# nmtrmail/Graphite

Hardware: AMD Instinct MI355X
Metric: simulated mem accesses/sec (node) at 1024 tiles, 1/2/4/8 GPU; bit-exact stats (higher is better)
Workload: dtype u64; 1 GPU; configs[3]: 1024 tiles (32x32 mesh) x 256 accesses per tile of the hotspot trace (20% to 256 lines shared by all tiles, WRITE p=1/3, ~2-cycle gaps), pr_l1_pr_l2_dram_directory_msi + full-map directory + DRAM history-tree queue + emesh_hop_by_hop (history-tree router contention), quantum 1000 ns, 8 logical shards (2-D blocks) over 1 GPU(s); tiles=1024, accesses_per_tile=256, hot_lines=256, mode=coherent, network=hop_by_hop

## Files before the change

graphite_amd/csrc/gg_coh_dev.h:

```cpp
#pragma once
#include "gg_dev.h"

#include <algorithm>
#include <type_traits>
#include <cmath>
#include <cstring>
#include <cstdlib>
#include <vector>

#ifndef GG_COH_DIAG
#define GG_COH_DIAG 0
#endif
#define DG(x) (GG_COH_DIAG ? (x) : nullptr)

namespace ggc {
using namespace gg;

enum { M_EX_REQ = GG_MSG_EX_REQ, M_SH_REQ = GG_MSG_SH_REQ, M_INV_REQ = GG_MSG_INV_REQ,
       M_FLUSH_REQ = GG_MSG_FLUSH_REQ, M_WB_REQ = GG_MSG_WB_REQ, M_EX_REP = GG_MSG_EX_REP,
       M_SH_REP = GG_MSG_SH_REP, M_INV_REP = GG_MSG_INV_REP, M_FLUSH_REP = GG_MSG_FLUSH_REP,
       M_WB_REP = GG_MSG_WB_REP, M_NULLIFY_REQ = GG_MSG_NULLIFY_REQ };
enum { DS_UNCACHED = 0, DS_SHARED = 1, DS_MODIFIED = 2, DS_OWNED = 3  };
enum { ST_I = 0, ST_S = 1, ST_M = 2, ST_O = 3  };
enum { M_UPGRADE_REP = GG_MSG_UPGRADE_REP, M_IFC_REQ = GG_MSG_INV_FLUSH_COMBINED_REQ };
enum { M_DRAM_FETCH_REQ = GG_MSG_DRAM_FETCH_REQ, M_DRAM_STORE_REQ = GG_MSG_DRAM_STORE_REQ,
       M_DRAM_FETCH_REP = GG_MSG_DRAM_FETCH_REP,
       M_DOWNGRADE_REQ = GG_MSG_DOWNGRADE_REQ, M_SH_REP_EX = GG_MSG_SH_REP_EX,
       M_DOWNGRADE_REP = GG_MSG_DOWNGRADE_REP };
constexpr uint32_t ST_E = ST_O;
enum { P_SELF = 0, P_LEFT, P_RIGHT, P_DOWN, P_UP, P_INJ };
#define INV_ADDR (~0ull)
#define NO_ENT (-0x7fffffff)

__device__ __forceinline__ bool to_directory(uint32_t t)
{
  return t == M_EX_REQ || t == M_SH_REQ || t == M_INV_REP || t == M_FLUSH_REP || t == M_WB_REP;
}
__device__ __forceinline__ bool has_data(uint32_t t)
{
  return t == M_EX_REP || t == M_SH_REP || t == M_FLUSH_REP || t == M_WB_REP ||
         t == M_DRAM_STORE_REQ || t == M_DRAM_FETCH_REP ||
         t == M_SH_REP_EX;
}
__device__ __forceinline__ uint32_t len_class(uint32_t t) { return has_data(t) ? 1u : t == M_IFC_REQ ? 2u : 0u; }

struct DEnt { uint64_t addr; int32_t owner; uint16_t dstate; uint16_t nsh; };
struct HMsg { uint64_t addr, arrival_ps; uint32_t type, src, requester, single_rx; };
struct TileSt { uint64_t rec, rec_end, clk, pend_start, out_addr, out_time; uint32_t blocked, seq, nrep, nrq; };
static_assert(sizeof(TileSt) == 64, "one 64-B line per tile");
struct CReq { uint64_t addr, time; uint32_t type, requester; };
struct CReqX { uint64_t arrival, start; uint32_t ds0, upg; int32_t sharer; uint32_t pad; };
constexpr uint32_t kCdl = 64;
constexpr uint64_t kRng0 = ((uint64_t)(uint32_t)GG_MOSI_RNG_SEED << 16) | 0x330Eu;
#define GG_LDS __attribute__((address_space(3)))
#define GG_GLB __attribute__((address_space(1)))
#if defined(__HIP_DEVICE_COMPILE__)
#define GG_DP __attribute__((address_space(1)))
#else
#define GG_DP
#endif
template <class D, class Q> inline void cs_set(D& dst, Q src) { dst = (D)src; }
struct Seg { uint32_t line, lo, hi, pad; };
enum { QS_Q = 0, QS_START, QS_DONE, QS_ARRIVED, QS_ACTIVE, QS_BLOCKED, QS_MIN_NEXT, QS_COUNT, QS_QPS,
       QS_BWAIT, QS_BMAX, QS_REL, QS_STOP, QS_N };
constexpr uint64_t kQsPaused = 4;
constexpr uint32_t kBarWait = 2;
__device__ __forceinline__ uint64_t rec_gap(uint32_t meta)
{
  return meta == GG_META_BARRIER ? 0ull : (uint64_t)((meta & 0x7FFFFFFFu) >> 1);
}

constexpr uint32_t kInLds = 512;
constexpr uint32_t kRqLds = 512;
constexpr uint32_t kChunks = 128;
constexpr uint32_t kChunk = 16;
constexpr uint32_t kQMax = 128;
constexpr uint32_t kNetCtr = 7;
constexpr size_t kWalkLdsMax = 160 * 1024;
constexpr uint32_t kWalkPkBytes = 5 * 8 + 7 * 4;

struct CP {
  uint32_t T, K, L;
  uint32_t s1, a1, s2, a2, log_line, pol1, pol2;
  uint32_t E, dassoc, log_dsets, log_slices, W, R, QC, IC;
  uint32_t bits_req, bits_data, bits_ifc, max_list, analytical, dram_qm, dram_qtype, dram_qaux;
  uint32_t net, nsx, nsy, mw, mh, qimg;
  uint32_t msg_cap, seg_cap, walk_pk;
  uint32_t seg_xcd;
  uint32_t cache_lds_off, cache_lds_bytes;
  uint32_t touch_each;
  uint32_t walk_wide;
  uint32_t no_hit_runs;
  uint32_t mt1, mt2, mt_log;
  uint32_t fast;
  uint32_t mosi;
  uint32_t shl2;
  uint32_t mesi;
  uint64_t lat_l1d, lat_l1t, lat_l2d, lat_l2t, lat_dir, gap_ps, dram_proc, dram_cost;
  NocParams np;
};

__device__ __forceinline__ uint32_t class_bits(const CP& P, uint32_t c) { return c == 1 ? P.bits_data : c == 2 ? P.bits_ifc : P.bits_req; }
__device__ __forceinline__ uint32_t msg_bits(const CP& P, uint32_t t) { return class_bits(P, len_class(t)); }

struct CS {
  GG_DP uint64_t* l1_tag; GG_DP uint8_t* l1_meta; GG_DP uint8_t* l1_rr;
  GG_DP uint64_t* l2_tag; GG_DP uint8_t* l2_meta; GG_DP uint8_t* l2_rr;
  GG_DP uint64_t* cc;
  GG_DP uint64_t* mtab;
  GG_DP unsigned long long* mtc;
  GG_DP uint64_t* st;
  GG_DP TileSt* ts;
  GG_DP DEnt* dir; GG_DP uint64_t* dsh;
  GG_DP DEnt* rep; GG_DP uint64_t* rsh;
  GG_DP CReq* rq;
  GG_DP CReqX* rqx;
  GG_DP uint64_t* drng; GG_DP uint64_t* rrng;
  GG_DP uint64_t* cdl; GG_DP uint32_t* ncdl;
  GG_DP uint64_t* ps;
  GG_DP HQueue* dq; GG_DP HNode* dnd;
  GG_DP const uint32_t* gtile; GG_DP const int32_t* ltile; GG_DP const uint32_t* shard;
  GG_DP const uint4* tinfo;
  GG_DP const uint64_t* addr; GG_DP const uint32_t* meta; GG_DP uint64_t* out;
  GG_DP gg_cmsg* pool0; GG_DP gg_cmsg* pool1; GG_DP uint32_t* npool;
  GG_DP uint32_t* inb0; GG_DP uint32_t* inb1;
  GG_DP uint32_t* arv0; GG_DP uint32_t* arv1;
  GG_DP uint32_t* cnt4;
  GG_DP uint64_t* xl; GG_DP uint32_t* nxl; GG_DP uint64_t* yl; GG_DP uint32_t* nyl;
  GG_DP const Seg* segx; GG_DP const Seg* segy;
  GG_DP const uint32_t* tseg;
  GG_DP gg_cmsg* bnd; GG_DP uint32_t* bnd_cnt;
// ... 2963 lines not shown
    r[20] = _hd; r[21] = _hl; r[22] = _hn;
    for (int i = 0; i < 9; ++i) r[23 + i] = T.tra[i];
  }
  if (T.rec >= T.rec_end) return kNsFin;
  if (T.blocked) return kNsBlk;
  return T.clk + rec_gap(S.meta[T.rec]) * P.gap_ps;
}


__device__ __forceinline__ void diag_off(CS& S)
{
  if (!GG_COH_DIAG) { S.prof = nullptr; S.trs = nullptr; S.trw = nullptr; S.tre = nullptr; }
}

#ifndef GG_KWARM
#define GG_KWARM 1
#endif
template <class A, class B>
__device__ __forceinline__ void kwarm(const A* __restrict__ a, const B* __restrict__ b)
{
  if (!GG_KWARM) return;
  const uint32_t* wa = reinterpret_cast<const uint32_t*>(a);
  const uint32_t* wb = reinterpret_cast<const uint32_t*>(b);
  constexpr uint32_t kA = (uint32_t)((sizeof(A) + 63) / 64), kB = (uint32_t)((sizeof(B) + 63) / 64);
  uint32_t x[kA + kB];
#pragma unroll
  for (uint32_t i = 0; i < kA; ++i) x[i] = wa[16 * i];
#pragma unroll
  for (uint32_t i = 0; i < kB; ++i) x[kA + i] = wb[16 * i];
  uint32_t acc = 0;
#pragma unroll
  for (uint32_t i = 0; i < kA + kB; ++i) acc ^= x[i];
  asm volatile("; kwarm %0" ::"s"(acc));
}

__device__ __forceinline__ void kt_begin(const CS& S)
{
  if (S.kt && threadIdx.x == 0)
    S.kt[(size_t)S.kt_slot * S.kt_stride + 2 * blockIdx.x] = __builtin_amdgcn_s_memrealtime();
}
__device__ __forceinline__ void kt_end(const CS& S)
{
  if (!S.kt) return;
  __syncthreads();
  if (threadIdx.x == 0) S.kt[(size_t)S.kt_slot * S.kt_stride + 2 * blockIdx.x + 1] = __builtin_amdgcn_s_memrealtime();
}


constexpr uint32_t kWalkSync = 512;
constexpr uint32_t kMaxWalkWaves = 16;
#ifndef GG_WALK_SLEEP
#define GG_WALK_SLEEP 1
#endif

__device__ __forceinline__ uint64_t wave_min64(uint64_t v)
{
#pragma unroll
  for (int o = 32; o > 0; o >>= 1) { const uint64_t u = (uint64_t)__shfl_xor((long long)v, o); v = u < v ? u : v; }
  return v;
}
__device__ __forceinline__ uint64_t lds_load_rlx(const uint64_t* p)
{
  return __hip_atomic_load(p, __ATOMIC_RELAXED, __HIP_MEMORY_SCOPE_WORKGROUP);
}
__device__ __forceinline__ void lds_store_rlx(uint64_t* p, uint64_t v)
{
  __hip_atomic_store(p, v, __ATOMIC_RELAXED, __HIP_MEMORY_SCOPE_WORKGROUP);
}

__device__ __forceinline__ uint64_t pipe_word(uint64_t t, uint32_t pos, uint32_t status)
{
  return (t << 12) | ((uint64_t)pos << 2) | status;
}
__device__ __forceinline__ uint32_t pipe_pos(uint64_t w) { return (uint32_t)(w >> 2) & 0x3FFu; }

struct WalkLds {
  uint64_t *Pt, *Ph, *Pk, *Pz;
  uint32_t *Pi, *Pp, *Pd, *Pf, *Pr;
  uint64_t *Qt; uint32_t *Qr, *Qs;
};

template <class Q>
__device__ __forceinline__ uint64_t serve_packet(const CP& P, const CS& S, const WalkLds& W, Q&& request, uint32_t i,
                                                 uint32_t nx, const Seg& sd, uint64_t zps, uint64_t& cf)
{
  const uint64_t t = W.Pt[i];
  const uint32_t f = W.Pf[i], nf = f & 0xFFFFFFu, d = W.Pd[i];
  const uint64_t qd = request(t, nf);
  cf += nf;
  uint32_t status = 0;
  if (nx < sd.lo || nx > sd.hi) status = 2;
  else if (nx == d) status = 1;
  W.Pt[i] = t + zps + lat_to_ps(qd, P.np.f);
  W.Pz[i] += zps;
  W.Pf[i] = nf | (status << 24);
  return qd;
}

__host__ __device__ inline bool walk_regq(const CP& P)
{
  return P.np.qm && P.np.qtype == GG_QM_HISTORY_TREE && P.np.max_size <= kQMax;
}

template <bool PIPE, bool RQ>
__device__ __forceinline__ void walk_body(const CP& P, const CS& S, uint32_t L, int stage, uint32_t blk, uint32_t qend = 0)
{
  uint32_t sg = blk;
  if (P.seg_xcd) {
    const uint32_t ns = P.seg_xcd, b = blk;
    sg = 2 * ((b % ns) + ns * (b / (2 * ns))) + ((b / ns) & 1u);
  }
  const uint32_t tid = threadIdx.x, nthr = blockDim.x, ln = tid & 63;
  const uint32_t wv = (uint32_t)__builtin_amdgcn_readfirstlane((int)(tid >> 6));
  uint32_t* cntp = (stage == 0 ? S.nxl : S.nyl) + sg;
  const uint64_t* list = (stage == 0 ? S.xl : S.yl) + (size_t)sg * P.seg_cap;
  const uint32_t live = S.live[L & 3];
  const uint32_t n0 = *cntp;
  const Seg sd = (stage == 0 ? S.segx : S.segy)[sg >> 1];
  const uint64_t lw = tid < P.seg_cap ? list[tid] : 0ull;
  uint32_t sent = 1;
  uint64_t qe_q = 0, qe_Q = 0;
  if (qend) {
    const uint32_t r0 = S.ring[0], r1 = S.ring[1], r2 = S.ring[2], r3 = S.ring[3], i0 = S.imp[0], i1 = S.imp[1];
    qe_q = S.qs[QS_Q]; qe_Q = S.qs[QS_COUNT];
    const uint32_t k = live - 1, km = k & 3;
    sent = (km == 0 ? r0 : km == 1 ? r1 : km == 2 ? r2 : r3) + (k == 0 ? ((qe_Q & 1) ? i1 : i0) : 0u);
  }
  if (!live) return;
  if (sent == 0) { quantum_end_walk(P, S, L, qe_q, qe_Q, blk, qend); return; }
  const uint32_t p = (live - 1) & 1u;
  PROF_T0();
  if (n0 == 0) return;
  const uint32_t n = min(n0, P.seg_cap);
  const uint32_t dir = sg & 1u;
  const int port = stage == 0 ? (dir ? P_RIGHT : P_LEFT) : (dir ? P_UP : P_DOWN);
  auto tile_at = [&](uint32_t pos) -> uint32_t { return stage == 0 ? sd.line * P.mw + pos : pos * P.mw + sd.line; };
  auto pos_of = [&](uint32_t tile) -> uint32_t { return stage == 0 ? tile % P.mw : tile / P.mw; };
  gg_cmsg* cur = pool(S, p);
  extern __shared__ __attribute__((aligned(16))) uint8_t smem[];
  const uint32_t npos = sd.hi - sd.lo + 1;
  const bool qm = RQ || P.np.qm != 0;
  constexpr bool regq = RQ;
  const bool sweep = !PIPE || n > 128 || P.walk_wide;
  const bool direct = PIPE && regq && !sweep;
  RegQueue rq;
  RegQueue::Raw rqr;
  const bool rq_direct = direct && wv < npos;
  const uint64_t rq_qi = rq_direct ? (uint64_t)tile_at(dir ? sd.lo + wv : sd.hi - wv) * 6 + port : 0ull;
  uint8_t* qimg = smem;
  uint64_t* lc = reinterpret_cast<uint64_t*>(smem + (size_t)npos * P.qimg);
  uint32_t* rlohi = reinterpret_cast<uint32_t*>(lc + (size_t)npos * kNetCtr);
  uint8_t* pk = reinterpret_cast<uint8_t*>(rlohi) + kWalkSync;
  if (n > P.walk_pk) { if (tid == 0) { atomicOr(S.err, GG_DERR_CAP); *cntp = 0; } return; }
  WalkLds W;
  W.Pt = reinterpret_cast<uint64_t*>(pk);
  W.Ph = W.Pt + P.walk_pk; W.Pk = W.Ph + P.walk_pk; W.Pz = W.Pk + P.walk_pk;
  W.Pi = reinterpret_cast<uint32_t*>(W.Pz + P.walk_pk);
  W.Pp = W.Pi + P.walk_pk; W.Pd = W.Pp + P.walk_pk; W.Pf = W.Pd + P.walk_pk;
  W.Pr = W.Pf + P.walk_pk;
  W.Qt = reinterpret_cast<uint64_t*>(W.Pr + P.walk_pk);
  W.Qr = reinterpret_cast<uint32_t*>(W.Qt + P.walk_pk); W.Qs = W.Qr + P.walk_pk;
  uint32_t pdst = 0, pf = 0;
  bool pheld = false;
  uint64_t haddr = 0;
  uint32_t hreq = 0, htype = 0, hlink = 0, hsrx = 0;
  const bool has_p = tid < n;
  const uint32_t orec = has_p ? (uint32_t)lw : 0u;
  pdst = has_p ? (uint32_t)(lw >> 32) : 0u;
  const gg_cmsg& om = cur[orec];
  const uint64_t ot = om.arrival_ps, os = om.send_ps, oz = om.zero_load_ps;
  const uint32_t osrc = om.src, oseq = om.seq, ohop = om.hop, otype = om.type;
  haddr = om.addr; hreq = om.requester; hlink = om.link; hsrx = om.single_rx;
  {
    const uint32_t z = pos_of(pdst);
    pheld = has_p && (z < sd.lo || z > sd.hi);
    const uint32_t hx = tile_at(z);
    pf = hx == pdst ? (uint32_t)S.ltile[pdst] : S.tseg[(size_t)hx * 2 + 1];
  }
  if (rq_direct) rqr = RegQueue::issue(S.nq + rq_qi, S.nnd + rq_qi * P.np.max_size, P.np.max_size, ln);
  if (tid < n) {
    const uint32_t i = tid;
    htype = otype;
    W.Pt[i] = ot; W.Ph[i] = os; W.Pk[i] = ((uint64_t)osrc << 32) | oseq; W.Pz[i] = oz;
    W.Pi[i] = orec; W.Pp[i] = pos_of(ohop); W.Pd[i] = pos_of(pdst);
    if (ot >> 51) atomicOr(S.err, GG_DERR_CAP);
    W.Pf[i] = (uint32_t)nflits(P.np, msg_bits(P, otype));
  }
// ... 59 lines not shown
    uint8_t* im = qimg + (size_t)(pos - sd.lo) * P.qimg;
    tr = HTree{reinterpret_cast<HQueue*>(im), reinterpret_cast<HNode*>(im + sizeof(HQueue)), 1, P.np.analytical != 0};
    if (regq) rq.load(tr.q, tr.nd, 1, P.np.analytical != 0, ln);
  };
  auto add_ctr = [&](uint32_t pos, uint64_t cq, uint64_t m, uint64_t cf) {
    uint64_t* l = lc + (size_t)(pos - sd.lo) * kNetCtr;
    l[0] += qm ? cq : 0; l[1] += qm ? m : 0; l[2] += cf; l[3] += m; l[4] += cf; l[5] += cf;
  };
  if (sweep && wv == 0) {
    uint64_t* K = W.Qt; uint32_t* B = W.Qr; uint32_t* O = W.Qs;
    for (uint32_t s_ = 0; lo <= hi && s_ <= hi - lo; ++s_) {
      const uint32_t pos = dir ? lo + s_ : hi - s_;
      uint32_t m = 0;
      for (uint32_t b0 = 0; b0 < n; b0 += 64) {
        const uint32_t i = b0 + ln;
        const bool at = i < n && W.Pp[i] == pos && (W.Pf[i] >> 24) == 0;
        const uint64_t bm = __ballot(at);
        if (at) {
          const uint32_t k = m + (uint32_t)__builtin_popcountll(bm & ((1ull << ln) - 1));
          B[k] = i; K[k] = (W.Pt[i] << 12) | W.Pr[i];
        }
        m += (uint32_t)__builtin_popcountll(bm);
      }
      if (m == 0) continue;
      wave_sync();
      for (uint32_t k = ln; k < m; k += 64) {
        const uint64_t kk = K[k];
        uint32_t r = 0;
        for (uint32_t j = 0; j < m; ++j) r += K[j] < kk;
        O[r] = B[k];
      }
      wave_sync();
      RegQueue rq; HTree tr;
      port_queue(pos, rq, tr);
      auto request = [&](uint64_t t, uint32_t nf) -> uint64_t {
        if (!qm) return 0;
        const uint64_t tc = time_to_cycles(t, P.np.f);
        return regq ? rq.request<false>(tc, nf, S.err) : (wave_q ? tr.delay_w(tc, nf, S.err, ln) : tr.delay(tc, nf, S.err));
      };
      const uint32_t nx = dir ? pos + 1 : pos - 1;
      uint64_t cq = 0, cf = 0;
      for (uint32_t k = 0; k < m; ++k) {
        const uint32_t i = O[k];
        cq += serve_packet(P, S, W, request, i, nx, sd, zps, cf);
        if (ln == 0) W.Pp[i] = nx;
        wave_sync();
      }
      nev += m;
      if (regq) rq.store(tr.q, tr.nd);
      if (ln == 0) add_ctr(pos, cq, m, cf);
      wave_sync();
    }
  } else if (!sweep && wv < npos) {
    const uint32_t pos = dir ? sd.lo + wv : sd.hi - wv;
    const uint32_t nx = dir ? pos + 1 : pos - 1;
    constexpr uint64_t kInf = ~0ull;
    const bool visited = lo <= hi && pos >= lo && pos <= hi;
    HTree tr;
    if (visited && !direct) port_queue(pos, rq, tr);
    const uint32_t status_nx = (nx < sd.lo || nx > sd.hi) ? 2u : 0u;
    const uint64_t zk = zps << 12;
    uint64_t cq = 0, cf = 0, m = 0;
    uint32_t spin = 0, polls = 0;
    const bool tev = DG(S.tre) && L >= kTrEv0 && L < kTrEv0 + S.tre_n;
    unsigned long long* tre = tev ? DG(S.tre) + (((size_t)(L - kTrEv0) * 2 + stage) * S.tr_wb + blk) * (kTrEvMax * 4 + 4) : nullptr;
    auto crosses = [&](uint32_t i) {
      if (i >= n) return false;
      const uint32_t a = W.Pp[i], z = W.Pd[i];
      return dir ? (a <= pos && pos < z) : (a >= pos && pos > z);
    };
    bool c0 = visited && crosses(ln), c1 = visited && crosses(ln + 64);
    const uint32_t r0 = c0 ? W.Pr[ln] : 0u, r1 = c1 ? W.Pr[ln + 64] : 0u;
    const uint32_t fd0 = c0 ? (W.Pf[ln] & 0xFFFFFFu) | (W.Pd[ln] << 24) : 0u;
    const uint32_t fd1 = c1 ? (W.Pf[ln + 64] & 0xFFFFFFu) | (W.Pd[ln + 64] << 24) : 0u;
    uint32_t go = visited ? 1u : 0u;
    uint64_t l0 = kInf, l1 = kInf;
    bool waiting = false;
    while (__builtin_amdgcn_readfirstlane((int)go)) {
      const uint64_t w0 = c0 ? lds_load_rlx(&W.Qt[ln]) : kInf;
      const uint64_t w1 = c1 ? lds_load_rlx(&W.Qt[ln + 64]) : kInf;
      if (waiting && !__ballot(w0 != l0 || w1 != l1)) {
        if (++spin > (1u << 22)) { if (ln == 0) atomicOr(S.err, GG_DERR_STATE); go = 0; continue; }
        __builtin_amdgcn_s_sleep(GG_WALK_SLEEP);
        continue;
      }
      waiting = false;
      l0 = w0; l1 = w1;
      uint64_t mk = kInf, bk = kInf;
      uint32_t mi = 0, mfd = 0;
      if (c0) {
        const uint32_t pp = pipe_pos(w0);
        const uint64_t k = (w0 & ~0xFFFull) | r0;
        if (pp == pos) { mk = k; mi = ln; mfd = fd0; }
        else bk = k + (uint64_t)(dir ? pos - pp : pp - pos) * zk;
      }
      if (c1) {
        const uint32_t pp = pipe_pos(w1);
        const uint64_t k = (w1 & ~0xFFFull) | r1;
        if (pp == pos) {
          if (k < mk) { mk = k; mi = ln + 64; mfd = fd1; }
        } else {
          const uint64_t b = k + (uint64_t)(dir ? pos - pp : pp - pos) * zk;
          bk = b < bk ? b : bk;
        }
      }
      uint64_t wk = kInf;
      uint32_t wl = 0;
      for (uint64_t bm = __ballot(mk != kInf); bm; bm &= bm - 1) {
        const uint32_t l = (uint32_t)__builtin_ctzll(bm);
        const uint64_t k = rl64(mk, l);
        if (k < wk) { wk = k; wl = l; }
      }
      const uint64_t below = __ballot(bk < wk);
      if (wk == kInf && !below) { go = 0; continue; }
      if (below) {
        if (++spin > (1u << 22)) { if (ln == 0) atomicOr(S.err, GG_DERR_STATE); go = 0; continue; }
        ++polls;
        waiting = true;
        __builtin_amdgcn_s_sleep(GG_WALK_SLEEP);
        continue;
      }
      const uint64_t T = wk >> 12;
      const uint64_t ev0 = tev ? __builtin_amdgcn_s_memtime() : 0;
      const uint32_t i = (uint32_t)__builtin_amdgcn_readlane((int)mi, (int)wl);
      const uint32_t fd = (uint32_t)__builtin_amdgcn_readlane((int)mfd, (int)wl);
      const uint32_t nf = fd & 0xFFFFFFu;
      const uint32_t status = status_nx ? status_nx : (nx == (fd >> 24) ? 1u : 0u);
      uint64_t evp = 0;
      auto pub = [&](uint64_t qd) {
        if (tev) evp = __builtin_amdgcn_s_memtime();
        if (ln == 0) lds_store_rlx(&W.Qt[i], pipe_word(T + zps + lat_to_ps(qd, P.np.f), nx, status));
      };
      uint64_t qd = 0;
      if (!qm) pub(0ull);
      else {
        const uint64_t tc = rfl64(time_to_cycles(T, P.np.f));
        if (regq) qd = rq.request_pub(tc, nf, pub);
        else { qd = wave_q ? tr.delay_w(tc, nf, S.err, ln) : tr.delay(tc, nf, S.err); pub(qd); }
      }
      const uint64_t ev1 = tev ? __builtin_amdgcn_s_memtime() : 0;
      cq += qd; cf += nf; ++m;
      if (ln == (i & 63)) { if (i < 64) c0 = false; else c1 = false; }
      if (tev && ln == 0) {
        const uint32_t k = atomicAdd(reinterpret_cast<unsigned int*>(&rlohi[2]), 1u);
        if (k < kTrEvMax) {
          unsigned long long* e = tre + 4 + 4 * k;
          e[0] = ev0; e[1] = evp; e[2] = ev1;
          e[3] = (unsigned long long)i | ((unsigned long long)pos << 16) | ((unsigned long long)wv << 24) |
                 ((unsigned long long)polls << 32);
        }
      }
      wave_sync();
    }
    if (regq && visited && direct && m) {
      const uint64_t qi = (uint64_t)tile_at(pos) * 6 + port;
      rq.errp = S.err; rq.store(S.nq + qi, S.nnd + qi * P.np.max_size);
    } else if (regq && visited && !direct) {
      rq.errp = S.err; rq.store(tr.q, tr.nd);
    }
    if (ln == 0 && visited) add_ctr(pos, cq, m, cf);
    nev = (uint32_t)m;
  }
  if (tid < n) {
    const uint32_t hx = tile_at(pos_of(pdst));
    pself = !pheld && hx == pdst;
    if (pheld) jres = atomicAdd(S.bnd_cnt, 1u);
    else if (pself) jres = atomicAdd(narv_at(S, p ^ 1u, pf), 1u);
    else { s2res = pf * 2 + (pdst / P.mw > hx / P.mw ? 1u : 0u); jres = atomicAdd(&S.nyl[s2res], 1u); }
  }
  __syncthreads();
  PROF_AT(_w2);
  uint32_t nb = 0;
  for (uint32_t i = tid; i < n; i += nthr) {
    const uint32_t r = W.Pi[i];
    uint32_t stt = W.Pf[i] >> 24, p1 = W.Pp[i];
    uint64_t ta = W.Pt[i], z = W.Pz[i];
    gg_cmsg* m = cur + r;
    if (!sweep) {
      const uint64_t w = W.Qt[i];
      const uint32_t p0 = p1;
      ta = w >> 12; p1 = pipe_pos(w); stt = (uint32_t)w & 3u;
      z += (uint64_t)(dir ? p1 - p0 : p0 - p1) * zps;
    }
    const uint32_t h = tile_at(p1);
    m->arrival_ps = ta; m->zero_load_ps = z; m->hop = h;
    const bool own = i == tid;
    if (stt == 2) {
      if (own && !pheld) { atomicOr(S.err, GG_DERR_STATE); continue; }
      const uint32_t j = own ? jres : atomicAdd(S.bnd_cnt, 1u);
      if (j >= P.msg_cap) { atomicOr(S.err, GG_DERR_CAP); continue; }
      gg_cmsg g;
      if (own) {
        const uint64_t kk = W.Pk[i];
        g.addr = haddr; g.send_ps = W.Ph[i]; g.src = (uint32_t)(kk >> 32); g.dst = pdst; g.requester = hreq;
        g.seq = (uint32_t)kk; g.type = htype; g.link = hlink; g.single_rx = hsrx;
      } else {
        g = *m;
      }
      g.arrival_ps = ta; g.zero_load_ps = z; g.hop = h;
      S.bnd[j] = g;
      ++nb;
      continue;
    }
    const uint32_t dst = own ? pdst : m->dst;
    if (own && (pheld || pself != (h == dst))) { atomicOr(S.err, GG_DERR_STATE); continue; }
// ... 198 lines not shown
```

graphite_amd/csrc/gg_coherent.hip:

```cpp
#include "gg_coh_many.h"
#include "gg_stats.h"
#include "gg_snapshot.h"

#include <algorithm>
#include <cmath>
#include <cstring>
#include <vector>

namespace ggc {

__global__ void k_c_import(CP P, CS S, const gg_cmsg* in, uint32_t n)
{
  const uint32_t i = blockIdx.x * blockDim.x + threadIdx.x;
  if (i >= n) return;
  import_one(P, S, in[i], &S.imp[0]);
}

__global__ void k_has_barrier(const uint32_t* meta, uint64_t n, uint32_t* flag)
{
  for (uint64_t i = (uint64_t)blockIdx.x * blockDim.x + threadIdx.x; i < n; i += (uint64_t)gridDim.x * blockDim.x)
    if (meta[i] == GG_META_BARRIER) { *flag = 1; return; }
}

__global__ void k_c_status(CP P, CS S, uint64_t* out )
// ... 936 lines not shown
    GG_HIP(hipGetLastError());
    uint64_t done = 0;
    uint32_t err = 0;
    GG_HIP(hipMemcpyAsync(&done, C->S.qs + QS_DONE, sizeof(done), hipMemcpyDeviceToHost, s));
    GG_HIP(hipMemcpyAsync(&err, ctx->err_dev, sizeof(err), hipMemcpyDeviceToHost, s));
    GG_HIP(hipStreamSynchronize(s));
    timed_harvest(C);
    if (err) break;
    if (done) break;
    if (batch < 256) batch *= 2;
  }
  gg_timer_end(ctx, "coherent_run", s);
  GG_HIP(hipStreamSynchronize(s));
  if (C->S.trs && getenv("GG_COH_TRACE_OUT")) {
    const std::string pre = getenv("GG_COH_TRACE_OUT");
    const size_t ns = (size_t)C->S.tr_n * P.L * kTrStep, nw = (size_t)C->S.tr_n * 2 * C->S.tr_wb * 8;
    std::vector<unsigned long long> h(std::max(ns, nw));
    for (int k = 0; k < 2; ++k) {
      const size_t cnt = k ? nw : ns;
      GG_HIP(hipMemcpy(h.data(), k ? C->S.trw : C->S.trs, 8 * cnt, hipMemcpyDeviceToHost));
      if (FILE* f = fopen((pre + (k ? ".walk" : ".step")).c_str(), "wb")) { fwrite(h.data(), 8, cnt, f); fclose(f); }
    }
    if (C->S.tre) {
      const size_t ne = (size_t)C->S.tre_n * 2 * C->S.tr_wb * (kTrEvMax * 4 + 4);
      std::vector<unsigned long long> he(ne);
      GG_HIP(hipMemcpy(he.data(), C->S.tre, 8 * ne, hipMemcpyDeviceToHost));
      if (FILE* f = fopen((pre + ".ev").c_str(), "wb")) { fwrite(he.data(), 8, ne, f); fclose(f); }
    }
    if (FILE* f = fopen((pre + ".meta").c_str(), "w")) {
      fprintf(f, "{\"launches\": %u, \"tiles\": %u, \"walk_blocks\": %u, \"nsx\": %u, \"nsy\": %u, \"wtx\": %u, \"wty\": %u, "
              "\"ev_first\": %u, \"ev_launches\": %u, \"ev_max\": %u}\n",
              C->S.tr_n, P.L, C->S.tr_wb, P.nsx, P.nsy, C->wtx, C->wty, kTrEv0, C->S.tre_n, kTrEvMax);
      fclose(f);
    }
  }
  if (C->S.prof) {
    std::vector<unsigned long long> h(1024 + 8 * 65536);
    GG_HIP(hipMemcpy(h.data(), C->S.prof, sizeof(unsigned long long) * h.size(), hipMemcpyDeviceToHost));
    unsigned long long crit = 0, wx = 0, wy = 0;
    for (int i = 0; i < 65536; ++i) { crit += h[1024 + i]; wx += h[1024 + 65536 + 2 * i]; wy += h[1024 + 65536 + 2 * i + 1]; }
    fprintf(stderr, "[gg_coh] step cycles over tiles: self %llu inbox+handlers %llu (order %llu) trace %llu publish %llu "
            "writeback %llu | slowest tile per launch %llu\n"
            "[gg_coh] walkers: %llu launches, staging %llu events %llu loop %llu handoff %llu, max events X %llu Y %llu | "
            "slowest walker per launch X %llu Y %llu | sweep: batch %llu queue load %llu requests %llu store %llu (s_memtime cycles); requests fast %llu M/G/1 %llu search %llu\n",
            h[0], h[1], h[9], h[2], h[3], h[4], crit, h[22], h[16], h[19], h[17], h[18], h[24], h[25], wx, wy, h[26], h[27], h[28], h[29], h[30], h[31], h[32]);
    {
      unsigned long long mt = 0, mx = 0, my = 0;
      for (int i = 0; i < 65536; ++i) { mt += h[1024 + 3 * 65536 + i]; mx += h[1024 + 4 * 65536 + 2 * i]; my += h[1024 + 4 * 65536 + 2 * i + 1]; }
      fprintf(stderr, "[gg_coh] tiles with SELF arrivals: %llu; cycles prologue %llu, narv %llu, gather %llu, order %llu, queue load %llu, "
              "requests + store %llu | tiles without: %llu, prologue %llu\n", h[96], h[90], h[91], h[92], h[93], h[94], h[95], h[98], h[97]);
      fprintf(stderr, "[gg_coh] per-launch max requests summed: tile (self+sent) %llu walker X %llu Y %llu\n", mt, mx, my);
      fprintf(stderr, "[gg_coh] walkers: most packets in one run X %llu Y %llu; pipelined runs past 64 packets (a lane's second "
              "candidate; past 128 wave 0 sweeps) %llu\n", h[46], h[47], h[48]);
      unsigned long long sn = 0, sa = 0, ss = 0, c1 = 0, c2 = 0, c3 = 0, ct = 0, nl = 0;
      for (int i = 0; i < 16384; ++i) {
        const unsigned long long* b = &h[1024 + 6 * 65536 + 4 * i];
        if (!b[0]) continue;
        ++nl; ct += b[0] >> 24;
        sn += (b[0] >> 16) & 255; sa += (b[0] >> 8) & 255; ss += b[0] & 255;
        c1 += (b[1] & 0xFFFFFF) << 8; c2 += (b[2] & 0xFFFFFF) << 8; c3 += (b[3] & 0xFFFFFF) << 8;
      }
      fprintf(stderr, "[gg_coh] slowest tile per launch (%llu launches, last 16384 indices): cycles %llu; inbox msgs %llu, SELF arrivals %llu, "
              "sent %llu; cycles self-phase %llu inbox+handlers %llu trace %llu\n", nl, ct, sn, sa, ss, c1, c2, c3);
      const char* kn[3] = {"SELF", "injection", "walker"};
      for (int k = 0; k < 3; ++k)
        fprintf(stderr, "[gg_coh] %s batches, requests by size 1|2-3|4-7|8-15|16-31|32-63|64+: %llu %llu %llu %llu %llu %llu %llu; tail requests %llu\n",
                kn[k], h[50 + 8 * k], h[51 + 8 * k], h[52 + 8 * k], h[53 + 8 * k], h[54 + 8 * k], h[55 + 8 * k], h[56 + 8 * k], h[80 + k]);
    }
    fprintf(stderr, "[gg_coh] trace: hit runs %llu cycles for %llu records (%llu calls, look-up part %llu; %llu row updates: "
            "loop %llu stores %llu); other accesses %llu cycles for %llu\n",
            h[33], h[34], h[38], h[37] - h[39], h[42], h[40] - h[37] + 0, h[41] - h[40], h[35], h[36]);
  }
  if (gg_status e = coh_check(ctx)) return e;
  uint64_t done = 0;
  GG_HIP(hipMemcpy(&done, C->S.qs + QS_DONE, sizeof(done), hipMemcpyDeviceToHost));
  *done_out = done;
  if (done == 2) return gg_fail(GG_ERR_STATE, "coherent run deadlocked: tiles blocked with no message in flight");
  return GG_OK;
}

static gg_status coh_owns_all(const gg_ctx* ctx, gg_status code, const char* what)
{
  const gg_config& c = ctx->cfg;
  const uint32_t K = c.num_shards ? c.num_shards : 1;
  if (c.shard_begin != 0 || (c.shard_end != 0 && c.shard_end != K))
    return gg_fail(code, "%s needs a context that owns every shard", what);
  return GG_OK;
}

gg_status gg_coherent_run(gg_ctx* ctx, const gg_trace* tr, uint64_t* access_out_dev, void* stream)
{
  GG_NOT_ATAC(ctx, "gg_coherent_run");
  if (!ctx) return gg_fail(GG_ERR_INVALID, "NULL argument");
  if (gg_status st = coh_owns_all(ctx, GG_ERR_INVALID, "gg_coherent_run")) return st;
  if (gg_status st = gg_coherent_begin(ctx, tr, access_out_dev, stream)) return st;
  uint64_t done = 0;
  return coh_drive(ctx, true, &done);
}

gg_status gg_coherent_advance(gg_ctx* ctx, uint64_t stop_quantum, uint64_t* next_quantum, int* done)
{
  GG_NOT_ATAC(ctx, "gg_coherent_advance");
  if (!ctx || !next_quantum || !done) return gg_fail(GG_ERR_INVALID, "NULL argument");
  if (gg_status st = coh_owns_all(ctx, GG_ERR_UNSUPPORTED, "gg_coherent_advance")) return st;
  gg_coh_state* C = ctx->coh;
  if (!C || !C->begun) return gg_fail(GG_ERR_INVALID, "gg_coherent_begin or gg_coherent_restore first");
// ... 605 lines not shown
```

graphite_amd/csrc/gg_dev.h:

```cpp
#pragma once
#include "gg_internal.h"

namespace gg {

struct HNode { uint64_t first, second; };
struct HQueue {
  uint32_t size; uint32_t max_size; uint32_t type, aux;
  uint64_t sig_sq, sig, n, newest;
  uint64_t analytical;
  uint64_t util, last_req, total_req;
  uint32_t front, back;
  double mean;
  uint64_t qtime;
  uint32_t head, pad;
};
static_assert(sizeof(HQueue) % 16 == 0 && sizeof(HNode) == 16, "16-byte queue images");

__host__ __device__ inline uint32_t hq_aux(uint32_t type, uint32_t basic_moving_avg, uint32_t list_no_interleaving)
{
  return type == GG_QM_BASIC ? basic_moving_avg : list_no_interleaving;
}
__host__ __device__ inline uint32_t hq_window(uint32_t aux) { return (aux & 0xFFFFu) ? (aux & 0xFFFFu) : 64u; }

inline gg_status gg_check_queue_model(uint32_t type, uint32_t aux, uint32_t max_size)
// ... 499 lines not shown
      } else {
        qd = la - t;
        if (lb - (la + p) >= min_proc) set(i1, la + p, lb);
        else --sz;
      }
    } else if (analytical && A(0) > t + p) {
      ++anl; ++n_anl;
      qd = mg1_queue_delay(nreq, newest, sig_sq, sig);
    } else {
      ++n_gen;
      const uint64_t tp = t + p;
      const uint64_t v0 = low_lanes(sz), v1 = sz > 64 ? low_lanes(sz - 64) : 0ull;
      const uint64_t le0 = cmp64<kCmpULE>(a0, t) & v0, le1 = cmp64<kCmpULE>(a1, t) & v1;
      const uint64_t f0 = le0 & cmp64<kCmpUGE>(b0, tp), f1 = le1 & cmp64<kCmpUGE>(b1, tp);
      const uint64_t l0 = ~le0 & v0 & cmp64<kCmpUGE>(b0 - a0, p), l1 = ~le1 & v1 & cmp64<kCmpUGE>(b1 - a1, p);
      const bool fit = (f0 | f1) != 0;
      const uint64_t m0 = fit ? f0 : l0, m1 = fit ? f1 : l1;
      const int i = m0 ? (int)__builtin_ctzll(m0) : (m1 ? 64 + (int)__builtin_ctzll(m1) : -1);
      if (i < 0) {
        errs |= GG_DERR_STATE;
      } else {
        const uint32_t ui = (uint32_t)i;
        const uint64_t a = A(ui), b = B(ui);
        if (t >= a) {
          if (t - a >= min_proc) {
            if (b - (t + p) >= min_proc) { shift_up(ui + 1); set(ui + 1, t + p, b); ++sz; }
            set(ui, a, t);
          } else if (b - (t + p) >= min_proc) {
            set(ui, t + p, b);
          } else {
            shift_down(ui); --sz;
          }
        } else {
          qd = a - t;
          if (b - (a + p) >= min_proc) set(ui, a + p, b);
          else { shift_down(ui); --sz; }
        }
      }
    }
    sig_sq += p * p;
    sig += p;
    if (sig_sq >= kMg1Exact || p >= (1ull << 26)) errs |= GG_DERR_RANGE;
    ++nreq;
    const uint64_t x = t + qd + p;
    newest = x > newest ? x : newest;
    util += p;
    last_req = x > last_req ? x : last_req;
    ++total_req;
    return qd;
  }
  __device__ __forceinline__ uint64_t rd64(uint64_t v) const { return rfl64(v); }
  __device__ __forceinline__ uint64_t A1(uint32_t i) const { return i < 64 ? rl64(a0, i) : rl64(a1, i - 64); }
  __device__ __forceinline__ uint64_t B1(uint32_t i) const { return i < 64 ? rl64(b0, i) : rl64(b1, i - 64); }
  template <class Pub>
  __device__ __forceinline__ uint64_t request_pub(uint64_t t, uint64_t p, Pub&& pub)
  {
    if (sz >= cap) { shift_down(0); --sz; }
    uint64_t qd = 0;
    const uint64_t tp = t + p;
    const uint64_t v0 = low_lanes(sz), v1 = sz > 64 ? low_lanes(sz - 64) : 0ull;
    const uint64_t le0 = cmp64<kCmpULE>(a0, t) & v0, le1 = cmp64<kCmpULE>(a1, t) & v1;
    const uint64_t f0 = le0 & cmp64<kCmpUGE>(b0, tp), f1 = le1 & cmp64<kCmpUGE>(b1, tp);
    if (f0 | f1) {
      pub(0ull);
      ++n_gen;
      const uint32_t ui = f0 ? (uint32_t)__builtin_ctzll(f0) : 64u + (uint32_t)__builtin_ctzll(f1);
      const uint64_t a = A1(ui), b = B1(ui);
      if (t - a >= min_proc) {
        if (b - tp >= min_proc) { shift_up(ui + 1); set(ui + 1, tp, b); ++sz; }
        set(ui, a, t);
      } else if (b - tp >= min_proc) {
        set(ui, tp, b);
      } else {
        shift_down(ui); --sz;
      }
    } else if (analytical && (cmp64<kCmpUGT>(a0, tp) & 1ull)) {
      qd = mg1_queue_delay(nreq, newest, sig_sq, sig);
      pub(qd);
      ++anl; ++n_anl;
    } else {
      ++n_gen;
      const uint64_t m0 = ~le0 & v0 & cmp64<kCmpUGE>(b0 - a0, p);
      const uint64_t m1 = ~le1 & v1 & cmp64<kCmpUGE>(b1 - a1, p);
      if ((m0 | m1) == 0) {
        pub(0ull);
        errs |= GG_DERR_STATE;
      } else {
        const uint32_t ui = m0 ? (uint32_t)__builtin_ctzll(m0) : 64u + (uint32_t)__builtin_ctzll(m1);
        const uint64_t a = A1(ui);
        qd = a - t;
        pub(qd);
        const uint64_t b = B1(ui);
        if (b - (a + p) >= min_proc) set(ui, a + p, b);
        else { shift_down(ui); --sz; }
      }
    }
    sig_sq = rd64(sig_sq + p * p);
    sig = rd64(sig + p);
    if (sig_sq >= kMg1Exact || p >= (1ull << 26)) errs |= GG_DERR_RANGE;
    nreq = rd64(nreq + 1);
    const uint64_t x = t + qd + p;
    newest = rd64(x > newest ? x : newest);
    util = rd64(util + p);
    last_req = rd64(x > last_req ? x : last_req);
    total_req = rd64(total_req + 1);
    anl = rd64(anl);
    sz = (uint32_t)__builtin_amdgcn_readfirstlane((int)sz);
    return qd;
  }
};

__device__ __forceinline__ uint64_t lat_to_ps(uint64_t cycles, double f)
{
  if (f == 1.0 && cycles < (1ull << 42)) return 1000 * cycles;
  return (uint64_t)ceil(((double)1000 * cycles) / f);
}
__device__ __forceinline__ uint64_t time_to_cycles(uint64_t ps, double f)
{
  if (f == 1.0 && ps < (1ull << 52)) return (ps + 999) / 1000;
  return (uint64_t)ceil(((double)ps * f) / 1.0e3);
}

struct NocParams {
  uint32_t tiles, w, h, flit_width, router_delay, link_delay, qm, analytical, max_size, net_model;
  uint32_t qtype, qaux;
  double f;
};

__device__ __forceinline__ uint64_t nflits(const NocParams& P, uint32_t bits)
{
  return (bits % P.flit_width == 0) ? bits / P.flit_width : bits / P.flit_width + 1;
}

__device__ __forceinline__ void cadd(uint64_t* c, uint32_t tile, int k, uint64_t v)
{
  if (v) atomicAdd((unsigned long long*)&c[(uint64_t)tile * GG_NUM_NET_COUNTERS + k], (unsigned long long)v);
}


__device__ __forceinline__ uint64_t route_closed_form(const NocParams& P, uint32_t s, uint32_t d, uint32_t bits,
                                                      uint64_t t, uint64_t& zl, uint64_t* ctr)
{
  zl = 0;
  if (s == d) return t;
  if (P.net_model == GG_NET_MAGIC) {
    cadd(ctr, s, GG_NC_PACKETS_SENT, 1); cadd(ctr, s, GG_NC_BITS_SENT, bits);
    const uint64_t l = lat_to_ps(1, P.f);
    t += l; zl += l;
    cadd(ctr, d, GG_NC_PACKETS_RECEIVED, 1); cadd(ctr, d, GG_NC_BITS_RECEIVED, bits);
    cadd(ctr, d, GG_NC_TOTAL_LATENCY_PS, zl);
    return t;
  }
  const uint64_t nf = nflits(P, bits);
  cadd(ctr, s, GG_NC_PACKETS_SENT, 1); cadd(ctr, s, GG_NC_FLITS_SENT, nf); cadd(ctr, s, GG_NC_BITS_SENT, bits);
  const int sx = (int)(s % P.w), sy = (int)(s / P.w), dx = (int)(d % P.w), dy = (int)(d / P.w);
  const uint64_t hops = (uint64_t)(abs(sx - dx) + abs(sy - dy));
  const uint64_t lat = lat_to_ps(hops * ((uint64_t)P.router_delay + P.link_delay), P.f);
  t += lat; zl += lat;
  cadd(ctr, s, GG_NC_BUFFER_WRITES, nf * hops); cadd(ctr, s, GG_NC_BUFFER_READS, nf * hops);
  cadd(ctr, s, GG_NC_SWITCH_ALLOC, hops); cadd(ctr, s, GG_NC_CROSSBAR, nf * hops);
  cadd(ctr, s, GG_NC_LINK_TRAVERSALS, nf * hops);
// ... 25 lines not shown
```

Baseline: 451,000 accesses/s.

## Precompute speculative forward for blocked walker packet and arm on predicted word

In the pipelined per-wave router walker, a wave blocked on an upstream packet used to sleep and re-poll the whole candidate set. Now, with register queues, it picks the earliest blocking packet, predicts the pipeline word that packet will have when it reaches this position, and runs the queue search for it in advance. It then spins on that one slot and publishes the forward word as soon as the prediction matches. The register queue request is split into prune/search/apply so the search can run before the publish and the update after. The goal is to shorten the serial hop-by-hop latency chain between neighbouring walker waves, at the cost of wasted searches when the prediction misses and a slightly smaller LDS budget.

Result: faster. 486,400 accesses/s (median of 6 runs) (+7.9%).

```diff
diff --git a/graphite_amd/csrc/gg_coh_dev.h b/graphite_amd/csrc/gg_coh_dev.h
--- a/graphite_amd/csrc/gg_coh_dev.h
+++ b/graphite_amd/csrc/gg_coh_dev.h
@@ -76,7 +76,7 @@
 constexpr uint32_t kChunk = 16;
 constexpr uint32_t kQMax = 128;
 constexpr uint32_t kNetCtr = 7;
-constexpr size_t kWalkLdsMax = 160 * 1024;
+constexpr size_t kWalkLdsMax = 160 * 1024 - 64;
 constexpr uint32_t kWalkPkBytes = 5 * 8 + 7 * 4;
 
 struct CP {
@@ -3146,6 +3146,9 @@
 #ifndef GG_WALK_SLEEP
 #define GG_WALK_SLEEP 1
 #endif
+#ifndef GG_WALK_ARM_SLEEP
+#define GG_WALK_ARM_SLEEP GG_WALK_SLEEP
+#endif
 
 __device__ __forceinline__ uint64_t wave_min64(uint64_t v)
 {
@@ -3226,7 +3229,7 @@
   PROF_T0();
   if (n0 == 0) return;
   const uint32_t n = min(n0, P.seg_cap);
-  const uint32_t dir = sg & 1u;
+  const uint32_t dir = (uint32_t)__builtin_amdgcn_readfirstlane((int)(sg & 1u));
   const int port = stage == 0 ? (dir ? P_RIGHT : P_LEFT) : (dir ? P_UP : P_DOWN);
   auto tile_at = [&](uint32_t pos) -> uint32_t { return stage == 0 ? sd.line * P.mw + pos : pos * P.mw + sd.line; };
   auto pos_of = [&](uint32_t tile) -> uint32_t { return stage == 0 ? tile % P.mw : tile / P.mw; };
@@ -3392,13 +3395,14 @@
       wave_sync();
     }
   } else if (!sweep && wv < npos) {
-    const uint32_t pos = dir ? sd.lo + wv : sd.hi - wv;
+    const uint32_t pos = (uint32_t)__builtin_amdgcn_readfirstlane((int)(dir ? sd.lo + wv : sd.hi - wv));
     const uint32_t nx = dir ? pos + 1 : pos - 1;
     constexpr uint64_t kInf = ~0ull;
     const bool visited = lo <= hi && pos >= lo && pos <= hi;
     HTree tr;
     if (visited && !direct) port_queue(pos, rq, tr);
-    const uint32_t status_nx = (nx < sd.lo || nx > sd.hi) ? 2u : 0u;
+    const uint32_t status_nx =
+        (uint32_t)__builtin_amdgcn_readfirstlane((int)((nx < sd.lo || nx > sd.hi) ? 2u : 0u));
     const uint64_t zk = zps << 12;
     uint64_t cq = 0, cf = 0, m = 0;
     uint32_t spin = 0, polls = 0;
@@ -3416,6 +3420,17 @@
     uint32_t go = visited ? 1u : 0u;
     uint64_t l0 = kInf, l1 = kInf;
     bool waiting = false;
+    uint32_t d_arm = 0, d_hit = 0, d_cont = 0, d_miss = 0;
+    auto rec_ev = [&](uint64_t ev0, uint64_t evp, uint64_t ev1, uint32_t i, uint32_t npoll) {
+      if (ln != 0) return;
+      const uint32_t k = atomicAdd(reinterpret_cast<unsigned int*>(&rlohi[2]), 1u);
+      if (k < kTrEvMax) {
+        unsigned long long* e = tre + 4 + 4 * k;
+        e[0] = ev0; e[1] = evp; e[2] = ev1;
+        e[3] = (unsigned long long)i | ((unsigned long long)pos << 16) | ((unsigned long long)wv << 24) |
+               ((unsigned long long)npoll << 32);
+      }
+    };
     while (__builtin_amdgcn_readfirstlane((int)go)) {
       const uint64_t w0 = c0 ? lds_load_rlx(&W.Qt[ln]) : kInf;
       const uint64_t w1 = c1 ? lds_load_rlx(&W.Qt[ln + 64]) : kInf;
@@ -3427,12 +3442,12 @@
       waiting = false;
       l0 = w0; l1 = w1;
       uint64_t mk = kInf, bk = kInf;
-      uint32_t mi = 0, mfd = 0;
+      uint32_t mi = 0, mfd = 0, bi = 0, bfd = 0;
       if (c0) {
         const uint32_t pp = pipe_pos(w0);
         const uint64_t k = (w0 & ~0xFFFull) | r0;
         if (pp == pos) { mk = k; mi = ln; mfd = fd0; }
-        else bk = k + (uint64_t)(dir ? pos - pp : pp - pos) * zk;
+        else { bk = k + (uint64_t)(dir ? pos - pp : pp - pos) * zk; bi = ln; bfd = fd0; }
       }
       if (c1) {
         const uint32_t pp = pipe_pos(w1);
@@ -3441,7 +3456,7 @@
           if (k < mk) { mk = k; mi = ln + 64; mfd = fd1; }
         } else {
           const uint64_t b = k + (uint64_t)(dir ? pos - pp : pp - pos) * zk;
-          bk = b < bk ? b : bk;
+          if (b < bk) { bk = b; bi = ln + 64; bfd = fd1; }
         }
       }
       uint64_t wk = kInf;
@@ -3453,44 +3468,83 @@
       }
       const uint64_t below = __ballot(bk < wk);
       if (wk == kInf && !below) { go = 0; continue; }
+      uint32_t i = 0, nf = 0;
+      uint64_t tc = 0, qd = 0, ev0 = 0, evp = 0;
+      RegQueue::Found fs{0ull, 0u, RegQueue::kNone};
       if (below) {
         if (++spin > (1u << 22)) { if (ln == 0) atomicOr(S.err, GG_DERR_STATE); go = 0; continue; }
         ++polls;
-        waiting = true;
-        __builtin_amdgcn_s_sleep(GG_WALK_SLEEP);
-        continue;
-      }
-      const uint64_t T = wk >> 12;
-      const uint64_t ev0 = tev ? __builtin_amdgcn_s_memtime() : 0;
-      const uint32_t i = (uint32_t)__builtin_amdgcn_readlane((int)mi, (int)wl);
-      const uint32_t fd = (uint32_t)__builtin_amdgcn_readlane((int)mfd, (int)wl);
-      const uint32_t nf = fd & 0xFFFFFFu;
-      const uint32_t status = status_nx ? status_nx : (nx == (fd >> 24) ? 1u : 0u);
-      uint64_t evp = 0;
-      auto pub = [&](uint64_t qd) {
-        if (tev) evp = __builtin_amdgcn_s_memtime();
-        if (ln == 0) lds_store_rlx(&W.Qt[i], pipe_word(T + zps + lat_to_ps(qd, P.np.f), nx, status));
-      };
-      uint64_t qd = 0;
-      if (!qm) pub(0ull);
-      else {
-        const uint64_t tc = rfl64(time_to_cycles(T, P.np.f));
-        if (regq) qd = rq.request_pub(tc, nf, pub);
-        else { qd = wave_q ? tr.delay_w(tc, nf, S.err, ln) : tr.delay(tc, nf, S.err); pub(qd); }
-      }
+        if constexpr (RQ) {
+          uint64_t bs = kInf;
+          uint32_t bl = 0;
+          for (uint64_t bm = below; bm; bm &= bm - 1) {
+            const uint32_t l = (uint32_t)__builtin_ctzll(bm);
+            const uint64_t k = rl64(bk, l);
+            if (k < bs) { bs = k; bl = l; }
+          }
+          const uint32_t ci = (uint32_t)__builtin_amdgcn_readlane((int)bi, (int)bl);
+          const uint32_t cfd = (uint32_t)__builtin_amdgcn_readlane((int)bfd, (int)bl);
+          const uint32_t cr = (uint32_t)bs & 0xFFFu, nf_ = cfd & 0xFFFFFFu;
+          const uint64_t Tc = bs >> 12;
+          const uint64_t pred = pipe_word(Tc, pos, 0u);
+          const uint32_t status = status_nx ? status_nx : (nx == (cfd >> 24) ? 1u : 0u);
+          rq.prune();
+          const uint64_t tc_ = rfl64(time_to_cycles(Tc, P.np.f));
+          fs = rq.search(tc_, nf_);
+          fs.qd = rfl64(fs.qd);
+          const uint64_t fwd = pipe_word(Tc + zps + rfl64(lat_to_ps(fs.qd, P.np.f)), nx, status);
+          uint64_t seen = GG_COH_DIAG ? rl64(ci < 64 ? w0 : w1, bl) : 0;
+          if (GG_COH_DIAG) ++d_arm;
+          bool hit = false;
+          for (;;) {
+            const uint64_t w = rfl64(lds_load_rlx(&W.Qt[ci]));
+            if (w == pred) { hit = true; break; }
+            const uint32_t pp = pipe_pos(w);
+            const uint64_t b = ((w & ~0xFFFull) | cr) + (uint64_t)(dir ? pos - pp : pp - pos) * zk;
+            if (b != bs) break;
+            if (GG_COH_DIAG && w != seen) { seen = w; ++d_cont; }
+            if (++spin > (1u << 22)) { if (ln == 0) atomicOr(S.err, GG_DERR_STATE); go = 0; break; }
+            __builtin_amdgcn_s_sleep(GG_WALK_ARM_SLEEP);
+          }
+          if (!hit) { if (GG_COH_DIAG) ++d_miss; continue; }
+          if (GG_COH_DIAG) ++d_hit;
+          ev0 = tev ? __builtin_amdgcn_s_memtime() : 0;
+          if (ln == 0) lds_store_rlx(&W.Qt[ci], fwd);
+          if (tev) evp = __builtin_amdgcn_s_memtime();
+          i = ci; nf = nf_; tc = tc_; qd = fs.qd;
+        } else {
+          waiting = true;
+          __builtin_amdgcn_s_sleep(GG_WALK_SLEEP);
+          continue;
+        }
+      } else {
+        const uint64_t T = wk >> 12;
+        ev0 = tev ? __builtin_amdgcn_s_memtime() : 0;
+        i = (uint32_t)__builtin_amdgcn_readlane((int)mi, (int)wl);
+        const uint32_t fd = (uint32_t)__builtin_amdgcn_readlane((int)mfd, (int)wl);
+        nf = fd & 0xFFFFFFu;
+        const uint32_t status = status_nx ? status_nx : (nx == (fd >> 24) ? 1u : 0u);
+        auto pub = [&](uint64_t qd) {
+          if (tev) evp = __builtin_amdgcn_s_memtime();
+          if (ln == 0) lds_store_rlx(&W.Qt[i], pipe_word(T + zps + lat_to_ps(qd, P.np.f), nx, status));
+        };
+        if (!qm) pub(0ull);
+        else {
+          tc = rfl64(time_to_cycles(T, P.np.f));
+          if (regq) { rq.prune(); fs = rq.search(tc, nf); qd = fs.qd; pub(qd); }
+          else { qd = wave_q ? tr.delay_w(tc, nf, S.err, ln) : tr.delay(tc, nf, S.err); pub(qd); }
+        }
+      }
+      if (regq) rq.apply(tc, nf, fs);
       const uint64_t ev1 = tev ? __builtin_amdgcn_s_memtime() : 0;
       cq += qd; cf += nf; ++m;
       if (ln == (i & 63)) { if (i < 64) c0 = false; else c1 = false; }
-      if (tev && ln == 0) {
-        const uint32_t k = atomicAdd(reinterpret_cast<unsigned int*>(&rlohi[2]), 1u);
-        if (k < kTrEvMax) {
-          unsigned long long* e = tre + 4 + 4 * k;
-          e[0] = ev0; e[1] = evp; e[2] = ev1;
-          e[3] = (unsigned long long)i | ((unsigned long long)pos << 16) | ((unsigned long long)wv << 24) |
-                 ((unsigned long long)polls << 32);
-        }
-      }
+      if (tev) rec_ev(ev0, evp, ev1, i, polls);
       wave_sync();
+    }
+    if (RQ && DG(S.prof) && ln == 0 && d_arm) {
+      atomicAdd(&DG(S.prof)[100], (unsigned long long)d_arm); atomicAdd(&DG(S.prof)[101], (unsigned long long)d_hit);
+      atomicAdd(&DG(S.prof)[102], (unsigned long long)d_cont); atomicAdd(&DG(S.prof)[103], (unsigned long long)d_miss);
     }
     if (regq && visited && direct && m) {
       const uint64_t qi = (uint64_t)tile_at(pos) * 6 + port;
diff --git a/graphite_amd/csrc/gg_coherent.hip b/graphite_amd/csrc/gg_coherent.hip
--- a/graphite_amd/csrc/gg_coherent.hip
+++ b/graphite_amd/csrc/gg_coherent.hip
@@ -1012,6 +1012,9 @@
       fprintf(stderr, "[gg_coh] per-launch max requests summed: tile (self+sent) %llu walker X %llu Y %llu\n", mt, mx, my);
       fprintf(stderr, "[gg_coh] walkers: most packets in one run X %llu Y %llu; pipelined runs past 64 packets (a lane's second "
               "candidate; past 128 wave 0 sweeps) %llu\n", h[46], h[47], h[48]);
+      fprintf(stderr, "[gg_coh] walkers, armed waits: arms %llu hits %llu (%.1f %% of %llu serves) misses %llu; "
+              "same-bound continues %llu\n", h[100], h[101], h[19] ? 100.0 * (double)h[101] / (double)h[19] : 0.0, h[19],
+              h[103], h[102]);
       unsigned long long sn = 0, sa = 0, ss = 0, c1 = 0, c2 = 0, c3 = 0, ct = 0, nl = 0;
       for (int i = 0; i < 16384; ++i) {
         const unsigned long long* b = &h[1024 + 6 * 65536 + 4 * i];
diff --git a/graphite_amd/csrc/gg_dev.h b/graphite_amd/csrc/gg_dev.h
--- a/graphite_amd/csrc/gg_dev.h
+++ b/graphite_amd/csrc/gg_dev.h
@@ -575,19 +575,34 @@
   __device__ __forceinline__ uint64_t rd64(uint64_t v) const { return rfl64(v); }
   __device__ __forceinline__ uint64_t A1(uint32_t i) const { return i < 64 ? rl64(a0, i) : rl64(a1, i - 64); }
   __device__ __forceinline__ uint64_t B1(uint32_t i) const { return i < 64 ? rl64(b0, i) : rl64(b1, i - 64); }
-  template <class Pub>
-  __device__ __forceinline__ uint64_t request_pub(uint64_t t, uint64_t p, Pub&& pub)
+  enum : uint32_t { kFit = 0, kAnalytical = 1, kLater = 2, kNone = 3 };
+  struct Found { uint64_t qd; uint32_t ui, kind; };
+  __device__ __forceinline__ void prune()
   {
     if (sz >= cap) { shift_down(0); --sz; }
-    uint64_t qd = 0;
+  }
+  __device__ __forceinline__ Found search(uint64_t t, uint64_t p) const
+  {
     const uint64_t tp = t + p;
     const uint64_t v0 = low_lanes(sz), v1 = sz > 64 ? low_lanes(sz - 64) : 0ull;
     const uint64_t le0 = cmp64<kCmpULE>(a0, t) & v0, le1 = cmp64<kCmpULE>(a1, t) & v1;
     const uint64_t f0 = le0 & cmp64<kCmpUGE>(b0, tp), f1 = le1 & cmp64<kCmpUGE>(b1, tp);
-    if (f0 | f1) {
-      pub(0ull);
+    if (f0 | f1)
+      return Found{0ull, f0 ? (uint32_t)__builtin_ctzll(f0) : 64u + (uint32_t)__builtin_ctzll(f1), kFit};
+    if (analytical && (cmp64<kCmpUGT>(a0, tp) & 1ull))
+      return Found{rd64(mg1_queue_delay(nreq, newest, sig_sq, sig)), 0u, kAnalytical};
+    const uint64_t m0 = ~le0 & v0 & cmp64<kCmpUGE>(b0 - a0, p);
+    const uint64_t m1 = ~le1 & v1 & cmp64<kCmpUGE>(b1 - a1, p);
+    if ((m0 | m1) == 0) return Found{0ull, 0u, kNone};
+    const uint32_t ui = m0 ? (uint32_t)__builtin_ctzll(m0) : 64u + (uint32_t)__builtin_ctzll(m1);
+    return Found{A1(ui) - t, ui, kLater};
+  }
+  __device__ __forceinline__ void apply(uint64_t t, uint64_t p, const Found& s)
+  {
+    const uint64_t tp = t + p, qd = s.qd;
+    const uint32_t ui = s.ui;
+    if (s.kind == kFit) {
       ++n_gen;
-      const uint32_t ui = f0 ? (uint32_t)__builtin_ctzll(f0) : 64u + (uint32_t)__builtin_ctzll(f1);
       const uint64_t a = A1(ui), b = B1(ui);
       if (t - a >= min_proc) {
         if (b - tp >= min_proc) { shift_up(ui + 1); set(ui + 1, tp, b); ++sz; }
@@ -597,26 +612,16 @@
       } else {
         shift_down(ui); --sz;
       }
-    } else if (analytical && (cmp64<kCmpUGT>(a0, tp) & 1ull)) {
-      qd = mg1_queue_delay(nreq, newest, sig_sq, sig);
-      pub(qd);
+    } else if (s.kind == kAnalytical) {
       ++anl; ++n_anl;
+    } else if (s.kind == kNone) {
+      ++n_gen;
+      errs |= GG_DERR_STATE;
     } else {
       ++n_gen;
-      const uint64_t m0 = ~le0 & v0 & cmp64<kCmpUGE>(b0 - a0, p);
-      const uint64_t m1 = ~le1 & v1 & cmp64<kCmpUGE>(b1 - a1, p);
-      if ((m0 | m1) == 0) {
-        pub(0ull);
-        errs |= GG_DERR_STATE;
-      } else {
-        const uint32_t ui = m0 ? (uint32_t)__builtin_ctzll(m0) : 64u + (uint32_t)__builtin_ctzll(m1);
-        const uint64_t a = A1(ui);
-        qd = a - t;
-        pub(qd);
-        const uint64_t b = B1(ui);
-        if (b - (a + p) >= min_proc) set(ui, a + p, b);
-        else { shift_down(ui); --sz; }
-      }
+      const uint64_t a = A1(ui), b = B1(ui);
+      if (b - (a + p) >= min_proc) set(ui, a + p, b);
+      else { shift_down(ui); --sz; }
     }
     sig_sq = rd64(sig_sq + p * p);
     sig = rd64(sig + p);
@@ -629,7 +634,6 @@
     total_req = rd64(total_req + 1);
     anl = rd64(anl);
     sz = (uint32_t)__builtin_amdgcn_readfirstlane((int)sz);
-    return qd;
   }
 };
 
```
